# xujiabo/SCREAM

Hardware: AMD Instinct MI355X
Metric: registration pairs/sec (higher is better)
Workload: dtype f32; 1 GPU; BASELINE configs[1]: synthetic 3DMatch_test-like pairs, voxel 0.0625 m, ~5k points/cloud, batch-of-pairs=32 per GPU, A1-A10 per pair (forward 6+6 layers d_model 256, 1-NN thresh 0.1, Kabsch, RE/TE), random-init weights seed 0; lanes=1, steps_in_flight=2, parallelism=dp1 (pairs sharded, metric-row all-gather), rccl_ranks=1, gemm_backend=h2

## Files before the change

scream_amd/csrc/ring.h:

```cpp
#pragma once
#include "split.h"

namespace {

constexpr int T_PF = 3;

typedef const __attribute__((address_space(1))) void* gptr_t;
typedef __attribute__((address_space(3))) void* lptr_t;

constexpr int TT = 256;
constexpr int T_SLOTS = 3;
constexpr int T_MAX_GRID = SCREAM_MAX_GRID;

template <class SP> constexpr int stage_bytes() { return SP::NP * 16 * 1024; }
template <class SP> constexpr int wave_pieces() { return SP::NP * 4; }

template <int N>
__device__ __forceinline__ void ring_barrier() {
    __builtin_amdgcn_s_waitcnt(0x0070 | (N & 15) | ((N >> 4) << 14));
    __builtin_amdgcn_s_barrier();
}

__device__ __forceinline__ void lds_only_barrier() {
    __builtin_amdgcn_s_waitcnt(0xC07F);
    __builtin_amdgcn_s_barrier();
}

__host__ __device__ __forceinline__ int chunk_k(int s2, int half, int j) { return 8 * (2 * s2 + (j >> 2)) + 4 * half + (j & 3); }

__device__ __forceinline__ f32x4 ld4(const float* p) { return *reinterpret_cast<const f32x4*>(p); }

__device__ __forceinline__ void dma_1k(const char* src_lane, char* dst, int k) {
    switch (k) {
        case 0: __builtin_amdgcn_global_load_lds((gptr_t)src_lane, (lptr_t)dst, 16, 0, 0); break;
        case 1: __builtin_amdgcn_global_load_lds((gptr_t)src_lane, (lptr_t)dst, 16, 1024, 0); break;
        case 2: __builtin_amdgcn_global_load_lds((gptr_t)src_lane, (lptr_t)dst, 16, 2048, 0); break;
        default: __builtin_amdgcn_global_load_lds((gptr_t)src_lane, (lptr_t)dst, 16, 3072, 0); break;
    }
}

template <class V>
__device__ __forceinline__ V ld_frag(const char* p) {
    return *reinterpret_cast<const V*>(p);
}

template <class SP, int NV = 0>
__device__ __forceinline__ void mfma_group(f32x16& acc, const typename SP::vec (&w)[SP::NP], const typename SP::vec (&a)[SP::NP],
                                           bool zero = false) {
    f32x16 z;
#pragma unroll
    for (int e = 0; e < 16; ++e) z[e] = 0.f;
    SP::products(acc, w, a, zero ? z : acc);
    if (NV < 0) return;
    __builtin_amdgcn_sched_group_barrier(0x008, 1, 0);
    __builtin_amdgcn_sched_group_barrier(0x100, SP::NP, 0);
    if (NV == 0) {
        if (SP::NPROD > 1) __builtin_amdgcn_sched_group_barrier(0x008, SP::NPROD - 1, 0);
    } else {
#pragma unroll
        for (int i = 0; i < SP::NPROD - 1; ++i) {
            __builtin_amdgcn_sched_group_barrier(0x002, NV, 0);
            __builtin_amdgcn_sched_group_barrier(0x008, 1, 0);
        }
        __builtin_amdgcn_sched_group_barrier(0x002, NV, 0);
    }
    __builtin_amdgcn_sched_barrier(0);
}

template <int STEP, bool NT = false>
__device__ __forceinline__ void ld_asm4(f32x4 (&d)[4], const void* sbase, unsigned voff) {
    static_assert(STEP == 1024 || STEP == 32, "");
    if (STEP == 1024 && NT) {
        asm volatile("global_load_dwordx4 %0, %1, %2 nt" : "=v"(d[0]) : "v"(voff), "s"(sbase));
        asm volatile("global_load_dwordx4 %0, %1, %2 offset:1024 nt" : "=v"(d[1]) : "v"(voff), "s"(sbase));
        asm volatile("global_load_dwordx4 %0, %1, %2 offset:2048 nt" : "=v"(d[2]) : "v"(voff), "s"(sbase));
        asm volatile("global_load_dwordx4 %0, %1, %2 offset:3072 nt" : "=v"(d[3]) : "v"(voff), "s"(sbase));
    } else if (STEP == 1024) {
        asm volatile("global_load_dwordx4 %0, %1, %2" : "=v"(d[0]) : "v"(voff), "s"(sbase));
        asm volatile("global_load_dwordx4 %0, %1, %2 offset:1024" : "=v"(d[1]) : "v"(voff), "s"(sbase));
        asm volatile("global_load_dwordx4 %0, %1, %2 offset:2048" : "=v"(d[2]) : "v"(voff), "s"(sbase));
        asm volatile("global_load_dwordx4 %0, %1, %2 offset:3072" : "=v"(d[3]) : "v"(voff), "s"(sbase));
    } else {
        asm volatile("global_load_dwordx4 %0, %1, %2" : "=v"(d[0]) : "v"(voff), "s"(sbase));
        asm volatile("global_load_dwordx4 %0, %1, %2 offset:32" : "=v"(d[1]) : "v"(voff), "s"(sbase));
        asm volatile("global_load_dwordx4 %0, %1, %2 offset:64" : "=v"(d[2]) : "v"(voff), "s"(sbase));
        asm volatile("global_load_dwordx4 %0, %1, %2 offset:96" : "=v"(d[3]) : "v"(voff), "s"(sbase));
    }
}
__device__ __forceinline__ void ld_asm2k(f32x4& d0, f32x4& d1, const void* sbase, unsigned voff) {
    asm volatile("global_load_dwordx4 %0, %1, %2" : "=v"(d0) : "v"(voff), "s"(sbase));
    asm volatile("global_load_dwordx4 %0, %1, %2 offset:1024" : "=v"(d1) : "v"(voff), "s"(sbase));
}
__device__ __forceinline__ void pin(f32x4& v) { asm volatile("" : "+v"(v)); }

#define VM_WAIT(N) asm volatile("s_waitcnt vmcnt(" #N ")" ::: "memory")
template <int N>
__device__ __forceinline__ void vm_wait() {
    static_assert(N == 0 || N == 4 || N == 8 || N == 12, "");
    if (N == 0) VM_WAIT(0);
    else if (N == 4) VM_WAIT(4);
    else if (N == 8) VM_WAIT(8);
    else VM_WAIT(12);
}

}
```

scream_amd/csrc/split.h:

```cpp
#pragma once
#include "common.h"

namespace {

typedef __bf16 bf16x8 __attribute__((ext_vector_type(8)));
typedef _Float16 f16x8 __attribute__((ext_vector_type(8)));

struct SplitBf3 {
    static constexpr int NP = 3;
    static constexpr int NPROD = 6;
    static constexpr bool SCALED = false;
    typedef bf16x8 vec;
    static __device__ __forceinline__ void split1(float x, int i, vec (&p)[3]) {
        const __bf16 a = (__bf16)x;
        const float r1 = x - (float)a;
        const __bf16 b = (__bf16)r1;
        p[0][i] = a;
        p[1][i] = b;
        p[2][i] = (__bf16)(r1 - (float)b);
    }
    static __device__ __forceinline__ f32x16 mfma(vec a, vec b, f32x16 c) { return __builtin_amdgcn_mfma_f32_32x32x16_bf16(a, b, c, 0, 0, 0); }
    template <bool MIRROR = false>
    static __device__ __forceinline__ void products(f32x16& acc, const vec (&x)[3], const vec (&y)[3], const f32x16& c0) {
        if (MIRROR) {
            acc = mfma(x[2], y[0], c0);
            acc = mfma(x[1], y[1], acc);
            acc = mfma(x[0], y[2], acc);
            acc = mfma(x[1], y[0], acc);
            acc = mfma(x[0], y[1], acc);
        } else {
            acc = mfma(x[0], y[2], c0);
            acc = mfma(x[1], y[1], acc);
            acc = mfma(x[2], y[0], acc);
            acc = mfma(x[0], y[1], acc);
            acc = mfma(x[1], y[0], acc);
        }
        acc = mfma(x[0], y[0], acc);
    }
};

struct SplitH2 {
    static constexpr int NP = 2;
    static constexpr int NPROD = 3;
    static constexpr bool SCALED = true;
    typedef f16x8 vec;
    static __device__ __forceinline__ void split1(float x, int i, vec (&p)[2]) {
        const _Float16 a = (_Float16)x;
        p[0][i] = a;
        p[1][i] = (_Float16)(x - (float)a);
    }
    static __device__ __forceinline__ void split1s(float x, float s, int i, vec (&p)[2]) {
        const _Float16 a = (_Float16)__builtin_fmaf(x, s, 0.0f);
        p[0][i] = a;
        p[1][i] = (_Float16)__builtin_fmaf(x, s, -(float)a);
    }
    static __device__ __forceinline__ void split2s(float x0, float x1, float s, int i, vec (&p)[2]) {
        typedef unsigned u32x4 __attribute__((ext_vector_type(4)));
        unsigned hi, lo;
        asm("v_fma_mixlo_f16 %0, %1, %2, 0" : "=v"(hi) : "v"(x0), "v"(s));
        asm("v_fma_mixhi_f16 %0, %1, %2, 0" : "+v"(hi) : "v"(x1), "v"(s));
        asm("v_fma_mixlo_f16 %0, %1, %2, -%3 op_sel_hi:[0,0,1]" : "=v"(lo) : "v"(x0), "v"(s), "v"(hi));
        asm("v_fma_mixhi_f16 %0, %1, %2, -%3 op_sel:[0,0,1] op_sel_hi:[0,0,1]" : "+v"(lo) : "v"(x1), "v"(s), "v"(hi));
        u32x4 a = __builtin_bit_cast(u32x4, p[0]), b = __builtin_bit_cast(u32x4, p[1]);
        a[i >> 1] = hi;
        b[i >> 1] = lo;
        p[0] = __builtin_bit_cast(vec, a);
        p[1] = __builtin_bit_cast(vec, b);
    }
    static __device__ __forceinline__ void split1s_pair_here(float x, float y, float s, int i, vec (&p)[2], vec (&q)[2]) {
        typedef unsigned u32x4 __attribute__((ext_vector_type(4)));
        u32x4 pa = __builtin_bit_cast(u32x4, p[0]), pb = __builtin_bit_cast(u32x4, p[1]);
        u32x4 qa = __builtin_bit_cast(u32x4, q[0]), qb = __builtin_bit_cast(u32x4, q[1]);
        unsigned ph = pa[i >> 1], pl = pb[i >> 1], qh = qa[i >> 1], ql = qb[i >> 1];
        if ((i & 1) == 0) {
            asm volatile("v_fma_mixlo_f16 %0, %1, %2, 0" : "=v"(ph) : "v"(x), "s"(s));
            asm volatile("v_fma_mixlo_f16 %0, %1, %2, 0" : "=v"(qh) : "v"(y), "s"(s));
            asm volatile("v_fma_mixlo_f16 %0, %1, %2, -%3 op_sel_hi:[0,0,1]" : "=v"(pl) : "v"(x), "s"(s), "v"(ph));
            asm volatile("v_fma_mixlo_f16 %0, %1, %2, -%3 op_sel_hi:[0,0,1]" : "=v"(ql) : "v"(y), "s"(s), "v"(qh));
        } else {
            asm volatile("v_fma_mixhi_f16 %0, %1, %2, 0" : "+v"(ph) : "v"(x), "s"(s));
            asm volatile("v_fma_mixhi_f16 %0, %1, %2, 0" : "+v"(qh) : "v"(y), "s"(s));
            asm volatile("v_fma_mixhi_f16 %0, %1, %2, -%3 op_sel:[0,0,1] op_sel_hi:[0,0,1]" : "+v"(pl) : "v"(x), "s"(s), "v"(ph));
            asm volatile("v_fma_mixhi_f16 %0, %1, %2, -%3 op_sel:[0,0,1] op_sel_hi:[0,0,1]" : "+v"(ql) : "v"(y), "s"(s), "v"(qh));
        }
        pa[i >> 1] = ph;
        pb[i >> 1] = pl;
        qa[i >> 1] = qh;
        qb[i >> 1] = ql;
        p[0] = __builtin_bit_cast(vec, pa);
        p[1] = __builtin_bit_cast(vec, pb);
        q[0] = __builtin_bit_cast(vec, qa);
        q[1] = __builtin_bit_cast(vec, qb);
    }
    static __device__ __forceinline__ f32x16 mfma(vec a, vec b, f32x16 c) { return __builtin_amdgcn_mfma_f32_32x32x16_f16(a, b, c, 0, 0, 0); }
    template <bool MIRROR = false>
    static __device__ __forceinline__ void products(f32x16& acc, const vec (&x)[2], const vec (&y)[2], const f32x16& c0) {
        acc = mfma(x[0], y[1], c0);
        acc = mfma(x[1], y[0], acc);
        acc = mfma(x[0], y[0], acc);
    }
    static __device__ __forceinline__ f32x16 product(int i, const vec (&x)[2], const vec (&y)[2], const f32x16& c) {
        return i == 0 ? mfma(x[0], y[1], c) : i == 1 ? mfma(x[1], y[0], c) : mfma(x[0], y[0], c);
    }
};

struct SplitH1 {
    static constexpr int NP = 1;
    static constexpr int NPROD = 1;
    static constexpr bool SCALED = true;
    typedef f16x8 vec;
    static __device__ __forceinline__ void split1(float x, int i, vec (&p)[1]) { p[0][i] = (_Float16)x; }
    static __device__ __forceinline__ void split1s(float x, float s, int i, vec (&p)[1]) { p[0][i] = (_Float16)__builtin_fmaf(x, s, 0.0f); }
    static __device__ __forceinline__ void split2s(float x0, float x1, float s, int i, vec (&p)[1]) {
        split1s(x0, s, i, p);
        split1s(x1, s, i + 1, p);
    }
    static __device__ __forceinline__ f32x16 mfma(vec a, vec b, f32x16 c) { return __builtin_amdgcn_mfma_f32_32x32x16_f16(a, b, c, 0, 0, 0); }
    template <bool MIRROR = false>
    static __device__ __forceinline__ void products(f32x16& acc, const vec (&x)[1], const vec (&y)[1], const f32x16& c0) {
        acc = mfma(x[0], y[0], c0);
    }
    static __device__ __forceinline__ f32x16 product(int, const vec (&x)[1], const vec (&y)[1], const f32x16& c) { return mfma(x[0], y[0], c); }
};

template <class SP>
__device__ __forceinline__ void split8(const f32x4 lo, const f32x4 hi, typename SP::vec (&p)[SP::NP]) {
#pragma unroll
    for (int i = 0; i < 8; ++i) SP::split1(i < 4 ? lo[i] : hi[i - 4], i, p);
}

template <class SP>
__device__ __forceinline__ void split8s(const f32x4 lo, const f32x4 hi, float s, typename SP::vec (&p)[SP::NP]) {
    if constexpr (SP::SCALED) {
#pragma unroll
        for (int i = 0; i < 8; i += 2) SP::split2s(i < 4 ? lo[i] : hi[i - 4], i < 4 ? lo[i + 1] : hi[i - 3], s, i, p);
    } else {
        split8<SP>(lo, hi, p);
    }
}

static inline float exp2i(int e) {
    union { uint32_t u; float f; } v;
    v.u = (uint32_t)(e + 127) << 23;
    return v.f;
}

}
```

scream_amd/csrc/tail_split.hip:

```cpp
#include <type_traits>

#include "ring.h"

namespace {

constexpr int T_RIDE0 = 3;
constexpr int T_STASH = 3;
constexpr int T_DEFER_H2 = 2;

constexpr int TAIL_STAGES = 72;
constexpr int NEXT_Q_STAGES = 8;
constexpr int KV_PLANES_BYTES = 8 * 3 * 2 * 1024;
constexpr int KV_IMAGE_BYTES = KV_PLANES_BYTES + 8 * 32 * 4;

constexpr int KV_H2_HEAD_BYTES = 2 * 2 * 1024;
constexpr int KV_H2_SCALE_OFF = 8 * KV_H2_HEAD_BYTES;

struct HeadOps {
    f32x4 kv[6];
    f32x4 ks[4];
    f32x4 sc;
};

struct TailScales {
    float s_att;
    int e_q;
    int e_att;
    float c1;
    float eps1;
    float s_m1;
    float ch;
    float c2;
    float eps2;
    float s_y;
    float cq;
};

__device__ __forceinline__ constexpr int xadd_slot(int h, int g, int nd) {
    int n = 0;
    for (int c = 15 - nd; c >= 8; --c) {
        if ((c >> 1) == h - 1) continue;
        if (c == g) return n < 4 ? n : -1;
        ++n;
    }
    return -1;
}

template <class SP, bool NQ>
__global__ __launch_bounds__(TT, 1) void tail_kernel(const float* __restrict__ Q,
                                                     const char* __restrict__ kvimg,
                                                     const int32_t* __restrict__ tile_cloud, int kv_cloud_offset,
                                                     const int32_t* __restrict__ cloud_len,
                                                     const float* __restrict__ xres,
                                                     const char* __restrict__ Wimg,
                                                     const float* __restrict__ g1, const float* __restrict__ b1,
                                                     const float* __restrict__ g2, const float* __restrict__ b2,
                                                     float* __restrict__ y,
                                                     float* q_next,
                                                     int n_tiles, TailScales sc) {
    static_assert(!NQ || SP::SCALED, "the next-layer query projection is built for the fp16 splits");
    constexpr int N_STAGES = TAIL_STAGES + (NQ ? NEXT_Q_STAGES : 0);
    typedef typename SP::vec V;
    constexpr int NP = SP::NP;
    constexpr int STAGE = stage_bytes<SP>();
    constexpr int PIECES = wave_pieces<SP>();
    constexpr bool APPLY_H2 = SP::SCALED;
    constexpr int NV_MERGE = SP::NPROD >= 6 ? 6 : 8;
    constexpr int ND = SP::NPROD >= 6 ? 1 : T_DEFER_H2;
    constexpr int NG = 16 - ND;
    constexpr int NSTASH = NP == 2 ? T_STASH : 0;
    __shared__ __attribute__((aligned(16))) char smem[T_SLOTS * STAGE + 4096 + NSTASH * 16384];
    const int tid = threadIdx.x, lane = tid & 63;
    const int wave = __builtin_amdgcn_readfirstlane(tid >> 6);
    const int half = lane >> 5;
    float* lnp = reinterpret_cast<float*>(smem + T_SLOTS * STAGE);
    f32x4* stash = reinterpret_cast<f32x4*>(smem + T_SLOTS * STAGE + 4096 + wave * (NSTASH * 4096)) + lane;
    lnp[tid] = SP::SCALED ? g1[tid] * sc.s_m1 : g1[tid];
    lnp[256 + tid] = SP::SCALED ? b1[tid] * sc.s_m1 : b1[tid];
    lnp[512 + tid] = g2[tid];
    lnp[768 + tid] = b2[tid];
    const float eps1 = SP::SCALED ? sc.eps1 : 1e-5f, eps2 = SP::SCALED ? sc.eps2 : 1e-5f;
    const unsigned v_lane16 = lane * 16, v_half16 = half * 16;
    auto dma_piece = [&](unsigned q, int u) {
        const unsigned src = q % (unsigned)N_STAGES, slot = q % (unsigned)T_SLOTS;
        const char* sbase = Wimg + (size_t)src * STAGE + (wave * PIECES + (u & ~3)) * 1024;
        dma_1k(sbase + v_lane16, smem + slot * STAGE + (wave * PIECES + (u & ~3)) * 1024, u & 3);
    };
    unsigned q = 0;
#pragma unroll
    for (int u = 0; u < PIECES; ++u) dma_piece(0, u);
#pragma unroll
    for (int u = 0; u < PIECES; ++u) dma_piece(1, u);

    auto seg_base = [&](const float* base, int64_t grp, int seg) { return base + grp + seg * 1024; };
    auto req_q = [&](f32x4 (&qb)[4], int64_t grp, int h) {
        ld_asm4<1024, true>(qb, seg_base(Q, grp, h), v_lane16);
    };
    auto req_head = [&](HeadOps& o, const char* kvc, int h) {
        f32x4 (&kv4)[4] = reinterpret_cast<f32x4 (&)[4]>(o.kv[0]);
        if (APPLY_H2) {
            ld_asm4<1024>(kv4, kvc + h * KV_H2_HEAD_BYTES, v_lane16);
            asm volatile("global_load_dwordx4 %0, %1, %2" : "=v"(o.sc) : "v"(v_half16), "s"(kvc + KV_H2_SCALE_OFF + 32 * h));
        } else {
            const char* kp = kvc + h * (3 * 2 * 1024);
            ld_asm4<1024>(kv4, kp, v_lane16);
            ld_asm2k(o.kv[4], o.kv[5], kp + 4 * 1024, v_lane16);
        }
        ld_asm4<32>(o.ks, kvc + KV_PLANES_BYTES + 128 * h, v_half16);
    };
    auto req_x = [&](f32x4 (&xs)[4], int64_t grp, int blk, auto second) {
        ld_asm4<1024, decltype(second)::value>(xs, seg_base(xres, grp, blk), v_lane16);
    };
    auto pin_head = [&](HeadOps& o) {
#pragma unroll
        for (int a = 0; a < 4; ++a) pin(o.ks[a]);
#pragma unroll
        for (int f = 0; f < (APPLY_H2 ? 4 : 6); ++f) pin(o.kv[f]);
        if (APPLY_H2) pin(o.sc);
    };
    auto add_x4 = [&](f32x16& t, const f32x4 (&xs)[4], int a, float c) {
#pragma unroll
        for (int k = 0; k < 4; ++k) t[4 * a + k] = SP::SCALED ? __builtin_fmaf(xs[a][k], c, t[4 * a + k]) : t[4 * a + k] + xs[a][k];
    };
    auto pin_x = [&](f32x4 (&xs)[4]) {
#pragma unroll
        for (int a = 0; a < 4; ++a) pin(xs[a]);
    };
    auto add_x = [&](f32x16& t, const f32x4 (&xs)[4], float c) {
#pragma unroll
        for (int a = 0; a < 4; ++a) add_x4(t, xs, a, c);
    };

    HeadOps op;
    f32x4 qA[4], qB[4];
    f32x4 xs[4], xs2[4];
    V apA[2][NP], apB[2][NP];
    f32x16 aT;
    bf16x8 qp[2][3];
    f16x8 qph[2][2];
    float Zs = 0.f;
    int tq = 0;

    auto apply_qscale = [&](const f32x4 (&qb)[4]) {
        float m = 0.f;
#pragma unroll
        for (int a = 0; a < 4; ++a)
#pragma unroll
            for (int k = 0; k < 4; ++k) m = fmaxf(m, qb[a][k]);
        m = fmaxf(m, __shfl_xor(m, 32));
        const int hb = (int)(__float_as_uint(op.sc[0]) >> 23);
        tq = min(max(14 - ((int)(__float_as_uint(m) >> 23) - 127), sc.e_q), min(127, sc.e_att + hb - 1));
    };
    auto apply_qsplit = [&](f32x4 (&qb)[4], int s2) {
        const f32x4 lo = qb[2 * s2], hi = qb[2 * s2 + 1];
        if (APPLY_H2) split8s<SplitH2>(lo, hi, __uint_as_float((uint32_t)(tq + 127) << 23), qph[s2]);
        else split8<SplitBf3>(lo, hi, qp[s2]);
    };
    auto apply_mfma = [&](int s2) {
        if (APPLY_H2) {
            f16x8 w[2];
#pragma unroll
            for (int p = 0; p < 2; ++p) w[p] = __builtin_bit_cast(f16x8, op.kv[p * 2 + s2]);
            mfma_group<SplitH2, -1>(aT, w, qph[s2], s2 == 0);
        } else {
            bf16x8 w[3];
#pragma unroll
            for (int p = 0; p < 3; ++p) w[p] = __builtin_bit_cast(bf16x8, op.kv[p * 2 + s2]);
            mfma_group<SplitBf3, -1>(aT, w, qp[s2], s2 == 0);
        }
    };
    auto apply_z = [&](f32x4 (&qb)[4]) {
        float zp = 0.f;
#pragma unroll
        for (int a = 0; a < 4; ++a)
#pragma unroll
            for (int k = 0; k < 4; ++k) zp += qb[a][k] * op.ks[a][k];
        zp += __shfl_xor(zp, 32);
        Zs = 1.0f / (zp + 1e-6f);
        if (APPLY_H2) Zs *= __uint_as_float((uint32_t)(sc.e_att - tq + (int)(__float_as_uint(op.sc[0]) >> 23)) << 23);
        else if (SP::SCALED) Zs *= sc.s_att;
    };
    auto apply_split_pair = [&](int k, V (&ap)[2][NP], float S) {
        const int s2 = k >> 2, j = (2 * k) & 7;
#pragma unroll
        for (int e = 0; e < 2; ++e) SP::split1((aT[2 * k + e] * Zs) * S, j + e, ap[s2]);
    };
    auto apply_ride = [&](f32x4 (&qb)[4], int g, V (&ap)[2][NP], float S) {
        if (g == 0 && APPLY_H2) apply_qscale(qb);
        if (g == 0) apply_qsplit(qb, 0);
        if (g == 1) apply_qsplit(qb, 1);
        if (g == 1) apply_mfma(0);
        if (g == 2) apply_mfma(1);
        if (g == 3) apply_z(qb);
        if (g >= 4 && g < 12) apply_split_pair(g - 4, ap, S);
    };

    int tile = blockIdx.x;
    int64_t grp = ((int64_t)tile * 128 + wave * 32) * SCREAM_D_MODEL;
    const char* kvc = nullptr;
    float S = 1.f;
    if (tile < n_tiles) {
        const int cl = tile_cloud[tile] + kv_cloud_offset;
        kvc = kvimg + (size_t)cl * KV_IMAGE_BYTES;
        S = (float)cloud_len[cl];
    }
    if (tile < n_tiles) {
#pragma unroll
        for (int h = 0; h < 2; ++h) {
            req_q(qA, grp, h);
            req_head(op, kvc, h);
            VM_WAIT(0);
            pin_x(qA);
            pin_head(op);
#pragma unroll
            for (int g = 0; g < 12; ++g) apply_ride(qA, g, h == 0 ? apA : apB, S);
        }
    }

    while (tile < n_tiles) {
        V wfd[ND][NP];
        f32x16 acc[8];
        auto ring_groups = [&](auto flush, auto body) __attribute__((always_inline)) {
            const char* wb = smem + (q % T_SLOTS) * STAGE + lane * 16;
            V wf[T_PF][NP];
#pragma unroll
            for (int g0 = 0; g0 < T_PF - 1; ++g0)
#pragma unroll
                for (int p = 0; p < NP; ++p) wf[g0][p] = ld_frag<V>(wb + (p * 16 + g0) * 1024);
            flush();
#pragma unroll
            for (int g = 0; g < NG; ++g) {
                if (g + T_PF - 1 < 16) {
#pragma unroll
                    for (int p = 0; p < NP; ++p)
                        (g + T_PF - 1 >= NG ? wfd[g + T_PF - 1 - NG][p] : wf[(g + T_PF - 1) % T_PF][p]) = ld_frag<V>(wb + (p * 16 + g + T_PF - 1) * 1024);
                }
                body(g, wf[g % T_PF]);
            }
            ++q;
        };
        const int tile_next = tile + (int)gridDim.x;
        const bool has_next = tile_next < n_tiles;
        const int64_t grp_next = ((int64_t)(has_next ? tile_next : tile) * 128 + wave * 32) * SCREAM_D_MODEL;
        const char* kvc_next = kvc;
        float S_next = 1.f;
        if (has_next) {
            const int cl = tile_cloud[tile_next] + kv_cloud_offset;
            kvc_next = kvimg + (size_t)cl * KV_IMAGE_BYTES;
            S_next = (float)cloud_len[cl];
        }

        auto stage_merge = [&](auto hh, V (&ap)[2][NP], V (&ap_next)[2][NP], f32x4 (&q_cons)[4], f32x4 (&q_req)[4], auto flush) {
            constexpr int h = decltype(hh)::value;
            constexpr bool RIDE = h >= 1 && h <= 6;
            if (h == 0) { if (NQ) ring_barrier<0>(); else lds_only_barrier(); }
            else ring_barrier<PIECES>();
            __builtin_amdgcn_sched_barrier(0);
            f32x4 (&x_prev)[4] = (h & 1) ? xs : xs2;
            f32x4 (&x_req)[4] = (h & 1) ? xs2 : xs;
            if (h > 0) {
                pin_x(x_prev);
                if (h - 1 < NSTASH) {
#pragma unroll
                    for (int a = 0; a < 4; ++a) stash[((h - 1) * 4 + a) * 64] = x_prev[a];
                }
                if (RIDE) {
                    pin_head(op);
                    pin_x(q_cons);
                }
            }
            __builtin_amdgcn_sched_barrier(0);
            req_x(x_req, grp, h, std::false_type{});
            if (h + 2 < 8) req_q(q_req, grp, h + 2);
            if (h == 0) req_head(op, kvc, 2);
            __builtin_amdgcn_sched_barrier(0);
            ring_groups(flush, [&](int g, const V (&w)[NP]) __attribute__((always_inline)) {
                if (g == 4 && RIDE && h + 2 < 8) {
                    __builtin_amdgcn_sched_barrier(0);
                    req_head(op, kvc, h + 2);
                    __builtin_amdgcn_sched_barrier(0);
                }
                if (g >= 4 && g - 4 < PIECES) dma_piece(q + 2, g - 4);
                if (PIECES == 12 && g == 14) dma_piece(q + 2, 11);
                if (RIDE) apply_ride(q_cons, g, ap_next, S);
                if (h > 0) {
                    const int pc = xadd_slot(h, g, ND);
                    if (pc >= 0) add_x4(acc[h > 0 ? h - 1 : 0], x_prev, pc, sc.c1);
                }
                mfma_group<SP, (h > 0 ? NV_MERGE : 0)>(acc[g >> 1], w, ap[g & 1], h == 0 && (g & 1) == 0);
            });
        };
        constexpr std::integral_constant<bool, true> yes{};
        constexpr std::integral_constant<bool, false> no{};
#define HEAD(n) std::integral_constant<int, n>{}
        auto flush_none = [&]() {};
        auto flush_acc7 = [&](V (&b)[2][NP], bool first) {
#pragma unroll
            for (int i = 0; i < ND; ++i) mfma_group<SP, -1>(acc[7], wfd[i], b[(NG + i) & 1], first && ((NG + i) & 1) == 0);
        };
        auto flush_mergeA = [&]() { flush_acc7(apA, false); };
        auto flush_mergeB = [&]() { flush_acc7(apB, false); };
        auto flush_mergeA0 = [&]() { flush_acc7(apA, true); };
        stage_merge(HEAD(0), apA, apB, qB, qA, flush_none);
        stage_merge(HEAD(1), apB, apA, qA, qB, flush_mergeA0);
        stage_merge(HEAD(2), apA, apB, qB, qA, flush_mergeB);
        stage_merge(HEAD(3), apB, apA, qA, qB, flush_mergeA);
        stage_merge(HEAD(4), apA, apB, qB, qA, flush_mergeB);
        stage_merge(HEAD(5), apB, apA, qA, qB, flush_mergeA);
        stage_merge(HEAD(6), apA, apB, qB, qA, flush_mergeB);
        stage_merge(HEAD(7), apB, apA, qA, qB, flush_mergeA);
        flush_mergeB();
        vm_wait<PIECES>();
        pin_x(xs2);
        add_x(acc[7], xs2, sc.c1);

        V mp[16][NP];
        {
            float sum = 0.f;
#pragma unroll
            for (int b = 0; b < 8; ++b)
#pragma unroll
                for (int e = 0; e < 16; ++e) sum += acc[b][e];
            sum += __shfl_xor(sum, 32);
            const float mean = sum * (1.0f / 256.0f);
            float var = 0.f;
#pragma unroll
            for (int b = 0; b < 8; ++b)
#pragma unroll
                for (int e = 0; e < 16; ++e) {
                    acc[b][e] -= mean;
                    var += acc[b][e] * acc[b][e];
                }
            var += __shfl_xor(var, 32);
            const float rstd = 1.0f / sqrtf(var * (1.0f / 256.0f) + eps1);
            const float* gp = lnp + 4 * half;
            const float* bp = lnp + 256 + 4 * half;
#pragma unroll
            for (int b = 0; b < 8; ++b)
#pragma unroll
                for (int s2 = 0; s2 < 2; ++s2) {
                    f32x4 v[2];
#pragma unroll
                    for (int a2 = 0; a2 < 2; ++a2) {
                        const int a = 2 * s2 + a2;
                        const f32x4 g4 = ld4(gp + 32 * b + 8 * a), b4 = ld4(bp + 32 * b + 8 * a);
#pragma unroll
                        for (int k = 0; k < 4; ++k) v[a2][k] = acc[b][4 * a + k] * rstd * g4[k] + b4[k];
                    }
                    split8<SP>(v[0], v[1], mp[2 * b + s2]);
                }
        }

        f32x16 hT;
        V hpA[2][NP], hpB[2][NP];
        auto split_pair = [&](int k, V (&hout)[2][NP]) {
            const int s2 = k >> 2, j = (2 * k) & 7;
            float x0, x1;
            asm("v_max_f32 %0, 0, %1" : "=v"(x0) : "v"(hT[2 * k]));
            asm("v_max_f32 %0, 0, %1" : "=v"(x1) : "v"(hT[2 * k + 1]));
            if constexpr (SP::SCALED) {
                SP::split2s(x0, x1, sc.ch, j, hout[s2]);
            } else {
                SP::split1(x0, j, hout[s2]);
                SP::split1(x1, j + 1, hout[s2]);
            }
        };
        auto stage_up = [&](auto first, auto xload, auto flush) {
            constexpr int XLOAD = decltype(xload)::value;
            if (decltype(first)::value) ring_barrier<0>(); else ring_barrier<PIECES>();
            __builtin_amdgcn_sched_barrier(0);
            if (XLOAD >= 0 && XLOAD < NSTASH) {
#pragma unroll
                for (int a = 0; a < 4; ++a) xs[a] = stash[(XLOAD * 4 + a) * 64];
            } else if (XLOAD >= 0) req_x(xs, grp, XLOAD, std::true_type{});
            __builtin_amdgcn_sched_barrier(0);
            ring_groups(flush, [&](int g, const V (&w)[NP]) __attribute__((always_inline)) {
                if (g < PIECES) dma_piece(q + 2, g);
                mfma_group<SP>(hT, w, mp[g], g == 0);
            });
        };
        auto stage_down = [&](V (&hin)[2][NP], V (&hout)[2][NP], auto with_split, auto xadd, auto ride, auto flush) {
            constexpr int XADD = decltype(xadd)::value;
            constexpr int RIDE = decltype(ride)::value;
            ring_barrier<PIECES>();
            __builtin_amdgcn_sched_barrier(0);
            if (XADD == 0) {
                pin_x(xs);
#pragma unroll
                for (int a = 0; a < 4; ++a)
#pragma unroll
                    for (int k = 0; k < 4; ++k) acc[0][4 * a + k] = SP::SCALED ? xs[a][k] * sc.c2 : xs[a][k];
            } else if (XADD > 0) {
                pin_x(xs);
                add_x(acc[XADD > 0 ? XADD : 0], xs, sc.c2);
            }
            if (RIDE == 2) {
                pin_head(op);
                pin_x(qA);
            }
            __builtin_amdgcn_sched_barrier(0);
            if (RIDE == 1) {
                req_q(qA, grp_next, 0);
                req_head(op, kvc_next, 0);
            }
            __builtin_amdgcn_sched_barrier(0);
            ring_groups(flush, [&](int g, const V (&w)[NP]) __attribute__((always_inline)) {
                if (RIDE == 2 && g == 4) {
                    __builtin_amdgcn_sched_barrier(0);
                    req_q(qA, grp_next, 1);
                    req_head(op, kvc_next, 1);
                    __builtin_amdgcn_sched_barrier(0);
                }
                if (RIDE == 2) {
                    if (g >= 4 && g - 4 < PIECES) dma_piece(q + 2, g - 4);
                    if (PIECES == 12 && g == 14) dma_piece(q + 2, 11);
                } else {
                    if (g < PIECES) dma_piece(q + 2, g);
                }
                if (RIDE == 2) apply_ride(qA, g, apA, S_next);
                if (decltype(with_split)::value && (ND == 1 ? (g & 1) == 0 : (g >= T_RIDE0 && g < T_RIDE0 + 8))) split_pair(ND == 1 ? g >> 1 : g - T_RIDE0, hout);
                mfma_group<SP>(acc[g >> 1], w, hin[g & 1], XADD == 0 && g >= 2 && (g & 1) == 0);
            });
        };
        constexpr std::integral_constant<int, -1> none{};
        constexpr std::integral_constant<int, 0> ride0{};
        auto flush_up = [&]() {
#pragma unroll
            for (int i = 0; i < ND; ++i) mfma_group<SP, -1>(hT, wfd[i], mp[NG + i]);
        };
        auto flush_downA = [&]() { flush_acc7(hpA, false); };
        auto flush_downB = [&]() { flush_acc7(hpB, false); };
        auto flush_downA0 = [&]() { flush_acc7(hpA, true); };
        stage_up(yes, none, flush_none);
        flush_up();
#pragma unroll
        for (int k = 0; k < 8; ++k) split_pair(k, hpA);
#define PAIR(c, fl, flA)                                                                    \
        stage_up(no, HEAD((c) - 1), fl);                                        \
        stage_down(hpA, hpB, yes, HEAD((c) - 1), ride0, flush_up);  \
        stage_up(no, HEAD(c), flA);                                         \
        stage_down(hpB, hpA, yes, HEAD(c), ride0, flush_up);
        PAIR(1, flush_none, flush_downA0) PAIR(3, flush_downB, flush_downA) PAIR(5, flush_downB, flush_downA) PAIR(7, flush_downB, flush_downA)
#undef PAIR
        for (int c = 9; c < 31; c += 2) {
            stage_up(no, none, flush_downB);
            stage_down(hpA, hpB, yes, none, ride0, flush_up);
            stage_up(no, none, flush_downA);
            stage_down(hpB, hpA, yes, none, ride0, flush_up);
        }
        stage_up(no, none, flush_downB);
        stage_down(hpA, hpB, yes, none, HEAD(1), flush_up);
        stage_down(hpB, hpA, no, none, HEAD(2), flush_downA);
        flush_downB();
#undef HEAD
        VM_WAIT(0);
        if (has_next) {
            pin_head(op);
            pin_x(qA);
#pragma unroll
            for (int g = 0; g < 12; ++g) apply_ride(qA, g, apB, S_next);
        }

        V yp[NQ ? 16 : 1][NP];
        {
            float sum = 0.f;
#pragma unroll
            for (int b = 0; b < 8; ++b)
#pragma unroll
                for (int e = 0; e < 16; ++e) sum += acc[b][e];
            sum += __shfl_xor(sum, 32);
            const float mean = sum * (1.0f / 256.0f);
            float var = 0.f;
#pragma unroll
            for (int b = 0; b < 8; ++b)
#pragma unroll
                for (int e = 0; e < 16; ++e) {
                    acc[b][e] -= mean;
                    var += acc[b][e] * acc[b][e];
                }
            var += __shfl_xor(var, 32);
            const float rstd = 1.0f / sqrtf(var * (1.0f / 256.0f) + eps2);
            const float* gp = lnp + 512 + 4 * half;
            const float* bp = lnp + 768 + 4 * half;
            float* yg = y + grp + lane * 4;
#pragma unroll
            for (int b = 0; b < 8; ++b)
#pragma unroll
                for (int s2 = 0; s2 < 2; ++s2) {
                    f32x4 o2[2];
#pragma unroll
                    for (int a2 = 0; a2 < 2; ++a2) {
                        const int a = 2 * s2 + a2;
                        const f32x4 g4 = ld4(gp + 32 * b + 8 * a), b4 = ld4(bp + 32 * b + 8 * a);
                        f32x4 o;
#pragma unroll
                        for (int k = 0; k < 4; ++k) o[k] = acc[b][4 * a + k] * rstd * g4[k] + b4[k];
                        __builtin_nontemporal_store(o, reinterpret_cast<f32x4*>(yg + (b * 4 + a) * 256));
                        o2[a2] = o;
                    }
                    if (NQ) split8<SP>(o2[0] * sc.s_y, o2[1] * sc.s_y, yp[NQ ? 2 * b + s2 : 0]);
                }
        }
        if constexpr (NQ) {
            f32x16 hq[2];
            f32x4 oq[4];
            float* qg = q_next + grp + lane * 4;
            auto elu_pair = [&](int k, const f32x16& h) {
#pragma unroll
                for (int e = 0; e < 2; ++e) {
                    const int i = 2 * k + e;
                    const float x = h[i] * sc.cq;
                    oq[i >> 2][i & 3] = elu1(x);
                }
            };
            auto store_chunk = [&](int j) {
#pragma unroll
                for (int a = 0; a < 4; ++a) __builtin_nontemporal_store(oq[a], reinterpret_cast<f32x4*>(qg + (j * 4 + a) * 256));
            };
            constexpr int PP = (PIECES + NG - 9) / (NG - 8);
            auto stage_q = [&](auto jj) {
                constexpr int j = decltype(jj)::value;
                if (j == 0) lds_only_barrier(); else ring_barrier<PIECES>();
                __builtin_amdgcn_sched_barrier(0);
                auto flush_q = [&]() {
                    if (j > 0) {
#pragma unroll
                        for (int i = 0; i < ND; ++i) mfma_group<SP, -1>(hq[(j + 1) & 1], wfd[i], yp[NG + i]);
                    }
                };
                ring_groups(flush_q, [&](int g, const V (&w)[NP]) __attribute__((always_inline)) {
                    if (j > 0 && g < 8) elu_pair(g, hq[(j + 1) & 1]);
                    if (g == 8) {
                        __builtin_amdgcn_sched_barrier(0);
                        if (j > 0) store_chunk(j - 1);
                        __builtin_amdgcn_sched_barrier(0);
                    }
                    if (g >= 8) {
#pragma unroll
                        for (int u = (g - 8) * PP; u < (g - 7) * PP; ++u)
                            if (u < PIECES) dma_piece(q + 2, u);
                    }
                    mfma_group<SP, 8>(hq[j & 1], w, yp[g], g == 0);
                });
            };
            stage_q(std::integral_constant<int, 0>{});
            stage_q(std::integral_constant<int, 1>{});
            stage_q(std::integral_constant<int, 2>{});
            stage_q(std::integral_constant<int, 3>{});
            stage_q(std::integral_constant<int, 4>{});
            stage_q(std::integral_constant<int, 5>{});
            stage_q(std::integral_constant<int, 6>{});
            stage_q(std::integral_constant<int, 7>{});
#pragma unroll
            for (int i = 0; i < ND; ++i) mfma_group<SP, -1>(hq[1], wfd[i], yp[NG + i]);
#pragma unroll
            for (int k = 0; k < 8; ++k) elu_pair(k, hq[1]);
            store_chunk(7);
        }
        tile = tile_next;
        grp = ((int64_t)tile_next * 128 + wave * 32) * SCREAM_D_MODEL;
        kvc = kvc_next;
        S = S_next;
    }
    VM_WAIT(0);
}

__global__ __launch_bounds__(256) void act_layout_kernel(const float* __restrict__ src, float* __restrict__ dst, int to_frag) {
    __shared__ float tile[32][260];
    const int t = threadIdx.x;
    const float* s = src + (int64_t)blockIdx.x * 8192;
    float* d = dst + (int64_t)blockIdx.x * 8192;
#pragma unroll
    for (int i = 0; i < 8; ++i) {
        const int e = t + 256 * i;
        const f32x4 v = *reinterpret_cast<const f32x4*>(s + e * 4);
        int row, col;
        if (to_frag) {
            row = e >> 6, col = (e & 63) * 4;
        } else {
            const int ln = e & 63, a = (e >> 6) & 3, blk = e >> 8;
            row = ln & 31, col = 32 * blk + 8 * a + 4 * (ln >> 5);
        }
        *reinterpret_cast<f32x4*>(&tile[row][col]) = v;
    }
    __syncthreads();
#pragma unroll
    for (int i = 0; i < 8; ++i) {
        const int e = t + 256 * i;
        int row, col;
        if (to_frag) {
            const int ln = e & 63, a = (e >> 6) & 3, blk = e >> 8;
            row = ln & 31, col = 32 * blk + 8 * a + 4 * (ln >> 5);
        } else {
            row = e >> 6, col = (e & 63) * 4;
        }
        *reinterpret_cast<f32x4*>(d + e * 4) = *reinterpret_cast<const f32x4*>(&tile[row][col]);
    }
}

template <class SP>
__global__ void pack_tail_kernel(const float* __restrict__ Wm, const float* __restrict__ W1, const float* __restrict__ W2,
                                 const float* __restrict__ Wq_next, float s_wm, float s_w1, float s_w2, float s_wq,
                                 typename SP::vec* __restrict__ out) {
    const int t = blockIdx.x * blockDim.x + threadIdx.x;
    if (t >= (TAIL_STAGES + (Wq_next ? NEXT_Q_STAGES : 0)) * 16 * 64) return;
    const int lane = t & 63, frag = (t >> 6) & 15, stage = t >> 10;
    const int m = lane & 31, half = lane >> 5;
    float v[8];
    float s;
    if (stage < 8) {
        s = s_wm;
#pragma unroll
        for (int j = 0; j < 8; ++j) v[j] = Wm[(int64_t)(32 * (frag >> 1) + m) * 256 + 32 * stage + chunk_k(frag & 1, half, j)];
    } else if (stage >= TAIL_STAGES) {
        s = s_wq;
#pragma unroll
        for (int j = 0; j < 8; ++j) v[j] = Wq_next[(int64_t)(32 * (stage - TAIL_STAGES) + m) * 256 + 32 * (frag >> 1) + chunk_k(frag & 1, half, j)];
    } else {
        const int st = stage - 8;
        const bool up = st == 0 || (st < 63 && (st & 1));
        const int c = st == 0 ? 0 : st == 63 ? 31 : up ? (st + 1) / 2 : st / 2 - 1;
        s = up ? s_w1 : s_w2;
        if (up) {
#pragma unroll
            for (int j = 0; j < 8; ++j) v[j] = W1[(int64_t)(32 * c + m) * 256 + 32 * (frag >> 1) + chunk_k(frag & 1, half, j)];
        } else {
#pragma unroll
            for (int j = 0; j < 8; ++j) v[j] = W2[(int64_t)(32 * (frag >> 1) + m) * 1024 + 32 * c + chunk_k(frag & 1, half, j)];
        }
    }
    typename SP::vec p[SP::NP];
#pragma unroll
    for (int j = 0; j < 8; ++j) SP::split1(SP::SCALED ? v[j] * s : v[j], j, p);
#pragma unroll
    for (int pl = 0; pl < SP::NP; ++pl) out[(((int64_t)stage * SP::NP + pl) * 16 + frag) * 64 + lane] = p[pl];
}

constexpr int KVF_THREADS = 320;

template <bool H2>
__global__ __launch_bounds__(KVF_THREADS) void kv_finalize_image_kernel(const float* __restrict__ partial,
                                                                      const int32_t* __restrict__ cloud_row0,
                                                                      const int32_t* __restrict__ cloud_len, int64_t row_base,
                                                                      int cloud_begin, char* __restrict__ kvimg,
                                                                      int64_t partial_layer_stride, int64_t image_layer_stride) {
    constexpr int KV_ELEMS = (SCREAM_HEAD_DIM + 1) * SCREAM_HEAD_DIM;
    static_assert(KV_ELEMS % 4 == 0 && KV_ELEMS / 4 <= KVF_THREADS, "");
    __shared__ float wmax[KVF_THREADS / 64];
    const int i4 = threadIdx.x;
    const bool active = i4 < KV_ELEMS / 4;
    const int kvi = blockIdx.x / SCREAM_NHEAD, h = blockIdx.x % SCREAM_NHEAD;
    const int cloud = cloud_begin + kvi;
    partial += (int64_t)blockIdx.y * partial_layer_stride;
    kvimg += (int64_t)blockIdx.y * image_layer_stride;
    const int t0 = (int)((cloud_row0[cloud] - row_base) / SCREAM_ROW_TILE);
    const int nt = (cloud_len[cloud] + SCREAM_ROW_TILE - 1) / SCREAM_ROW_TILE;
    const float* p = partial + ((int64_t)t0 * SCREAM_NHEAD + h) * KV_ELEMS + 4 * (active ? i4 : 0);
    char* img = kvimg + (size_t)cloud * KV_IMAGE_BYTES;
    const float S = (float)cloud_len[cloud];
    f32x4 s8[16];
#pragma unroll
    for (int u = 0; u < 16; ++u) s8[u] = f32x4{0.f, 0.f, 0.f, 0.f};
    if (active) {
        for (int c = 0; c < nt; c += 16) {
#pragma unroll
            for (int u = 0; u < 16; ++u)
                if (c + u < nt) s8[u] += *reinterpret_cast<const f32x4*>(p + (int64_t)(c + u) * SCREAM_NHEAD * KV_ELEMS);
        }
    }
#pragma unroll
    for (int u = 0; u < 8; ++u) s8[u] += s8[u + 8];
    const f32x4 s4 = ((s8[0] + s8[1]) + (s8[2] + s8[3])) + ((s8[4] + s8[5]) + (s8[6] + s8[7]));
    const bool is_kv = 4 * i4 < 32 * 32;
    f32x4 x4;
#pragma unroll
    for (int e = 0; e < 4; ++e) x4[e] = s4[e] / S;
    float scale = 1.f;
    if (H2) {
        float m = (active && is_kv) ? fmaxf(fmaxf(fabsf(x4[0]), fabsf(x4[1])), fmaxf(fabsf(x4[2]), fabsf(x4[3]))) : 0.f;
#pragma unroll
        for (int o = 32; o >= 1; o >>= 1) m = fmaxf(m, __shfl_xor(m, o));
        if ((threadIdx.x & 63) == 0) wmax[threadIdx.x >> 6] = m;
        __syncthreads();
        m = wmax[0];
#pragma unroll
        for (int w = 1; w < KVF_THREADS / 64; ++w) m = fmaxf(m, wmax[w]);
        const uint32_t mb = __float_as_uint(m);
        int eh = 15 - ((int)(mb >> 23) - 127) - ((mb & 0x7fffffu) ? 1 : 0);
        if (!(m >= 1.17549435e-38f) || eh > 40) eh = 40;
        if (eh < -30) eh = -30;
        scale = __uint_as_float((uint32_t)(eh + 127) << 23);
        if (threadIdx.x < 8) reinterpret_cast<float*>(img + KV_H2_SCALE_OFF)[h * 8 + threadIdx.x] = __uint_as_float((uint32_t)(127 - eh) << 23);
    }
    if (!active) return;
#pragma unroll
    for (int e = 0; e < 4; ++e) {
        const int i = 4 * i4 + e;
        if (is_kv) {
            const int d = i >> 5, v = i & 31;
            const float x = x4[e];
            const int s2 = d >> 4, hf = (d >> 2) & 1, j = 4 * ((d >> 3) & 1) + (d & 3);
            if (H2) {
                const _Float16 a = (_Float16)(x * scale);
                const _Float16 b = (_Float16)__builtin_fmaf(x, scale, -(float)a);
                _Float16* base = reinterpret_cast<_Float16*>(img) + ((size_t)(h * 2) * 2 + s2) * 512 + (v + 32 * hf) * 8 + j;
                base[0] = a;
                base[2 * 512] = b;
            } else {
                const __bf16 a = (__bf16)x;
                const float r1 = x - (float)a;
                const __bf16 b = (__bf16)r1;
                const __bf16 cc = (__bf16)(r1 - (float)b);
                __bf16* base = reinterpret_cast<__bf16*>(img) + ((size_t)(h * 3) * 2 + s2) * 512 + (v + 32 * hf) * 8 + j;
                base[0] = a;
                base[2 * 512] = b;
                base[4 * 512] = cc;
            }
        } else {
            reinterpret_cast<float*>(img + KV_PLANES_BYTES)[h * 32 + (i - 32 * 32)] = s4[e];
        }
    }
}

bool split_ok(int32_t split) { return split == SCREAM_SPLIT_BF3 || split == SCREAM_SPLIT_H2 || split == SCREAM_SPLIT_H1; }

bool tail_scales(const scream_tail_exps_t* ex, TailScales* sc) {
    if (!ex) return false;
    const int es[6] = {ex->e_att, ex->e_wm, ex->e_m1, ex->e_w1, ex->e_h, ex->e_w2};
    for (int e : es)
        if (e < -40 || e > 40) return false;
    const int e1 = ex->e_wm + ex->e_att, e2 = ex->e_w2 + ex->e_h, eh = ex->e_h - ex->e_w1 - ex->e_m1;
    if (e1 < -44 || e1 > 44 || e2 < -44 || e2 > 44 || eh < -100 || eh > 100) return false;
    if (ex->e_q < -40 || ex->e_q > 40) return false;
    sc->s_att = exp2i(ex->e_att);
    sc->e_q = ex->e_q;
    sc->e_att = ex->e_att;
    sc->c1 = exp2i(e1);
    sc->eps1 = 1e-5f * exp2i(2 * e1);
    sc->s_m1 = exp2i(ex->e_m1);
    sc->ch = exp2i(eh);
    sc->c2 = exp2i(e2);
    sc->eps2 = 1e-5f * exp2i(2 * e2);
    if (ex->e_y < -40 || ex->e_y > 40 || ex->e_wq < -40 || ex->e_wq > 40) return false;
    sc->s_y = exp2i(ex->e_y);
    sc->cq = exp2i(-ex->e_y - ex->e_wq);
    return true;
}

}

extern "C" int64_t scream_tail_image_bytes(int32_t split, int32_t with_next_q) {
    if (!split_ok(split) || (with_next_q && split == SCREAM_SPLIT_BF3)) return SCREAM_EINVAL;
    return (int64_t)(TAIL_STAGES + (with_next_q ? NEXT_Q_STAGES : 0)) * split * 16 * 1024;
}
extern "C" int64_t scream_kv_image_bytes(void) { return KV_IMAGE_BYTES; }

extern "C" int scream_pack_tail(const float* Wm, const float* W1, const float* W2, const float* Wq_next, int32_t split,
                                const scream_tail_exps_t* exps, void* image, void* stream) {
    SCREAM_REQUIRE(Wm && W1 && W2 && image && split_ok(split), SCREAM_EINVAL);
    SCREAM_REQUIRE(!Wq_next || split != SCREAM_SPLIT_BF3, SCREAM_EUNSUPPORTED);
    SCREAM_REQUIRE((reinterpret_cast<uintptr_t>(image) & 15) == 0, SCREAM_EINVAL);
    const dim3 grid((TAIL_STAGES + (Wq_next ? NEXT_Q_STAGES : 0)) * 16 * 64 / 256), block(256);
    if (split != SCREAM_SPLIT_BF3) {
        TailScales sc;
        SCREAM_REQUIRE(tail_scales(exps, &sc), SCREAM_EINVAL);
        if (split == SCREAM_SPLIT_H2)
            pack_tail_kernel<SplitH2><<<grid, block, 0, as_stream(stream)>>>(Wm, W1, W2, Wq_next, exp2i(exps->e_wm), exp2i(exps->e_w1),
                                                                             exp2i(exps->e_w2), exp2i(exps->e_wq), reinterpret_cast<f16x8*>(image));
        else
            pack_tail_kernel<SplitH1><<<grid, block, 0, as_stream(stream)>>>(Wm, W1, W2, Wq_next, exp2i(exps->e_wm), exp2i(exps->e_w1),
                                                                             exp2i(exps->e_w2), exp2i(exps->e_wq), reinterpret_cast<f16x8*>(image));
    } else {
        pack_tail_kernel<SplitBf3><<<grid, block, 0, as_stream(stream)>>>(Wm, W1, W2, nullptr, 1.f, 1.f, 1.f, 1.f, reinterpret_cast<bf16x8*>(image));
    }
    SCREAM_LAUNCH_CHECK();
    return 0;
}

extern "C" int scream_kv_finalize_image(const float* kv_partial, const int32_t* cloud_row0, const int32_t* cloud_len,
                                        int64_t row_base, int32_t cloud_begin, int32_t n_kv, void* kv_image, int32_t n_layers,
                                        int64_t partial_layer_stride, int64_t image_layer_stride, int32_t split, void* stream) {
    SCREAM_REQUIRE(kv_partial && cloud_row0 && cloud_len && kv_image && split_ok(split), SCREAM_EINVAL);
    SCREAM_REQUIRE(n_kv >= 0 && cloud_begin >= 0 && row_base >= 0 && n_layers >= 1 && n_layers <= 65535, SCREAM_EINVAL);
    SCREAM_REQUIRE(n_layers == 1 || (partial_layer_stride > 0 && image_layer_stride > 0 && image_layer_stride % 16 == 0), SCREAM_EINVAL);
    SCREAM_REQUIRE(((reinterpret_cast<uintptr_t>(kv_image) | reinterpret_cast<uintptr_t>(kv_partial)) & 15) == 0 && partial_layer_stride % 4 == 0,
                   SCREAM_EINVAL);
    if (n_kv == 0) return 0;
    const dim3 grid(n_kv * SCREAM_NHEAD, n_layers), block(KVF_THREADS);
    if (split != SCREAM_SPLIT_BF3)
        kv_finalize_image_kernel<true><<<grid, block, 0, as_stream(stream)>>>(kv_partial, cloud_row0, cloud_len, row_base, cloud_begin,
                                                                              reinterpret_cast<char*>(kv_image), partial_layer_stride, image_layer_stride);
    else
        kv_finalize_image_kernel<false><<<grid, block, 0, as_stream(stream)>>>(kv_partial, cloud_row0, cloud_len, row_base, cloud_begin,
                                                                               reinterpret_cast<char*>(kv_image), partial_layer_stride, image_layer_stride);
    SCREAM_LAUNCH_CHECK();
    return 0;
}

namespace {
template <class SP, bool NQ>
void launch_tail(unsigned grid, hipStream_t st, const float* Q, const void* kv_image, const int32_t* tile_cloud, int32_t kv_cloud_offset,
                 const int32_t* cloud_len, const float* x, const void* tail_image, const float* g1, const float* b1, const float* g2,
                 const float* b2, float* y, float* q_next, int tiles, const TailScales& sc) {
    tail_kernel<SP, NQ><<<dim3(grid), dim3(TT), 0, st>>>(Q, reinterpret_cast<const char*>(kv_image), tile_cloud, kv_cloud_offset, cloud_len, x,
                                                     reinterpret_cast<const char*>(tail_image), g1, b1, g2, b2, y, q_next, tiles, sc);
}
}

extern "C" int scream_layer_tail_f32(const float* Q, const void* kv_image, const int32_t* tile_cloud,
                                     int32_t kv_cloud_offset, const int32_t* cloud_len, const float* x,
                                     const void* tail_image, const float* g1, const float* b1, const float* g2,
                                     const float* b2, float* y, float* q_next, int64_t M, int32_t split,
                                     const scream_tail_exps_t* exps, void* stream) {
    SCREAM_REQUIRE(Q && kv_image && tile_cloud && cloud_len && x && tail_image && g1 && b1 && g2 && b2 && y && split_ok(split), SCREAM_EINVAL);
    SCREAM_REQUIRE(M >= 0 && M % SCREAM_ROW_TILE == 0, SCREAM_EUNSUPPORTED);
    SCREAM_REQUIRE(((reinterpret_cast<uintptr_t>(Q) | reinterpret_cast<uintptr_t>(kv_image) | reinterpret_cast<uintptr_t>(x) |
                     reinterpret_cast<uintptr_t>(tail_image) | reinterpret_cast<uintptr_t>(g1) | reinterpret_cast<uintptr_t>(b1) |
                     reinterpret_cast<uintptr_t>(g2) | reinterpret_cast<uintptr_t>(b2) | reinterpret_cast<uintptr_t>(y) |
                     reinterpret_cast<uintptr_t>(q_next)) & 15) == 0, SCREAM_EINVAL);
    SCREAM_REQUIRE(x != y, SCREAM_EINVAL);
    SCREAM_REQUIRE(!q_next || (split != SCREAM_SPLIT_BF3 && q_next != x && q_next != y), SCREAM_EINVAL);
    TailScales sc{1.f, 0, 0, 1.f, 1e-5f, 1.f, 1.f, 1.f, 1e-5f, 1.f, 1.f};
    if (split != SCREAM_SPLIT_BF3) SCREAM_REQUIRE(tail_scales(exps, &sc), SCREAM_EINVAL);
    const int64_t tiles = M / SCREAM_ROW_TILE;
    if (tiles == 0) return 0;
    SCREAM_REQUIRE(tiles < (1ll << 31), SCREAM_EUNSUPPORTED);
    const unsigned grid = tiles < T_MAX_GRID ? (unsigned)tiles : (unsigned)T_MAX_GRID;
    hipStream_t st = as_stream(stream);
#define TAIL_ARGS grid, st, Q, kv_image, tile_cloud, kv_cloud_offset, cloud_len, x, tail_image, g1, b1, g2, b2, y, q_next, (int)tiles, sc
    if (split == SCREAM_SPLIT_H2) {
        if (q_next) launch_tail<SplitH2, true>(TAIL_ARGS);
        else launch_tail<SplitH2, false>(TAIL_ARGS);
    } else if (split == SCREAM_SPLIT_H1) {
        if (q_next) launch_tail<SplitH1, true>(TAIL_ARGS);
        else launch_tail<SplitH1, false>(TAIL_ARGS);
    } else {
        launch_tail<SplitBf3, false>(TAIL_ARGS);
    }
#undef TAIL_ARGS
    SCREAM_LAUNCH_CHECK();
    return 0;
}

extern "C" int scream_act_layout(const float* src, float* dst, int64_t M, int32_t to_fragment, void* stream) {
    SCREAM_REQUIRE(src && dst && src != dst, SCREAM_EINVAL);
    SCREAM_REQUIRE(M >= 0 && M % 32 == 0 && M / 32 < (1ll << 31), SCREAM_EUNSUPPORTED);
    SCREAM_REQUIRE(((reinterpret_cast<uintptr_t>(src) | reinterpret_cast<uintptr_t>(dst)) & 15) == 0, SCREAM_EINVAL);
    if (M == 0) return 0;
    act_layout_kernel<<<dim3((unsigned)(M / 32)), dim3(256), 0, as_stream(stream)>>>(src, dst, to_fragment ? 1 : 0);
    SCREAM_LAUNCH_CHECK();
    return 0;
}
```

Before: 1895 pairs/s.

## Interleave H2 split, x-add and fragment loads between individual MFMAs

For the SplitH2 backend, the down stage now issues each MFMA product separately, fenced by scheduling barriers. It slots the next fragment LDS loads, DMA issue, the residual x-add into the accumulators and a staged f16 hi/lo split of the activations between those MFMAs. The deferred flush products in flush_up get the same per-product placement. The goal is to hide VALU and LDS latency under the matrix pipe instead of running them as separate bursts. In exchange the compiler loses scheduling freedom, register pressure rises, and the hand ordering may stall if the dependencies are placed too tightly.

```diff
diff --git a/scream_amd/csrc/ring.h b/scream_amd/csrc/ring.h
--- a/scream_amd/csrc/ring.h
+++ b/scream_amd/csrc/ring.h
@@ -67,6 +67,18 @@
     __builtin_amdgcn_sched_barrier(0);
 }
 
+template <class SP, class Mfma, class Behind>
+__device__ __forceinline__ void mfma_group_placed(Mfma&& mfma, Behind&& behind) {
+#pragma unroll
+    for (int m = 0; m < SP::NPROD; ++m) {
+        __builtin_amdgcn_sched_barrier(0);
+        mfma(m);
+        __builtin_amdgcn_sched_barrier(0);
+        behind(m);
+    }
+    __builtin_amdgcn_sched_barrier(0);
+}
+
 template <int STEP, bool NT = false>
 __device__ __forceinline__ void ld_asm4(f32x4 (&d)[4], const void* sbase, unsigned voff) {
     static_assert(STEP == 1024 || STEP == 32, "");
diff --git a/scream_amd/csrc/split.h b/scream_amd/csrc/split.h
--- a/scream_amd/csrc/split.h
+++ b/scream_amd/csrc/split.h
@@ -37,6 +37,10 @@
         }
         acc = mfma(x[0], y[0], acc);
     }
+    static __device__ __forceinline__ f32x16 product(int i, const vec (&x)[3], const vec (&y)[3], const f32x16& c) {
+        return i == 0 ? mfma(x[0], y[2], c) : i == 1 ? mfma(x[1], y[1], c) : i == 2 ? mfma(x[2], y[0], c)
+             : i == 3 ? mfma(x[0], y[1], c) : i == 4 ? mfma(x[1], y[0], c) : mfma(x[0], y[0], c);
+    }
 };
 
 struct SplitH2 {
@@ -66,6 +70,22 @@
         b[i >> 1] = lo;
         p[0] = __builtin_bit_cast(vec, a);
         p[1] = __builtin_bit_cast(vec, b);
+    }
+    static __device__ __forceinline__ void split2s_step(int step, float x0, float x1, float s, unsigned& hi, unsigned& lo, int i, vec (&p)[2]) {
+        typedef unsigned u32x4 __attribute__((ext_vector_type(4)));
+        if (step == 0) {
+            asm volatile("v_fma_mixlo_f16 %0, %1, %2, 0" : "=v"(hi) : "v"(x0), "v"(s));
+        } else if (step == 1) {
+            asm volatile("v_fma_mixlo_f16 %0, %1, %2, -%3 op_sel_hi:[0,0,1]" : "=v"(lo) : "v"(x0), "v"(s), "v"(hi));
+            asm volatile("v_fma_mixhi_f16 %0, %1, %2, 0" : "+v"(hi) : "v"(x1), "v"(s));
+        } else {
+            asm volatile("v_fma_mixhi_f16 %0, %1, %2, -%3 op_sel:[0,0,1] op_sel_hi:[0,0,1]" : "+v"(lo) : "v"(x1), "v"(s), "v"(hi));
+            u32x4 a = __builtin_bit_cast(u32x4, p[0]), b = __builtin_bit_cast(u32x4, p[1]);
+            a[i >> 1] = hi;
+            b[i >> 1] = lo;
+            p[0] = __builtin_bit_cast(vec, a);
+            p[1] = __builtin_bit_cast(vec, b);
+        }
     }
     static __device__ __forceinline__ void split1s_pair_here(float x, float y, float s, int i, vec (&p)[2], vec (&q)[2]) {
         typedef unsigned u32x4 __attribute__((ext_vector_type(4)));
diff --git a/scream_amd/csrc/tail_split.hip b/scream_amd/csrc/tail_split.hip
--- a/scream_amd/csrc/tail_split.hip
+++ b/scream_amd/csrc/tail_split.hip
@@ -68,6 +68,7 @@
     constexpr int NV_MERGE = SP::NPROD >= 6 ? 6 : 8;
     constexpr int ND = SP::NPROD >= 6 ? 1 : T_DEFER_H2;
     constexpr int NG = 16 - ND;
+    constexpr bool PLACED = std::is_same<SP, SplitH2>::value;
     constexpr int NSTASH = NP == 2 ? T_STASH : 0;
     __shared__ __attribute__((aligned(16))) char smem[T_SLOTS * STAGE + 4096 + NSTASH * 16384];
     const int tid = threadIdx.x, lane = tid & 63;
@@ -239,6 +240,28 @@
             }
             ++q;
         };
+        auto ring_groups_placed = [&](auto flush, auto fride, auto mfma, auto ride) __attribute__((always_inline)) {
+            const char* wb = smem + (q % T_SLOTS) * STAGE + lane * 16;
+            V wf[T_PF][NP];
+#pragma unroll
+            for (int g0 = 0; g0 < T_PF - 1; ++g0)
+#pragma unroll
+                for (int p = 0; p < NP; ++p) wf[g0][p] = ld_frag<V>(wb + (p * 16 + g0) * 1024);
+            flush(fride);
+#pragma unroll
+            for (int g = 0; g < NG; ++g) {
+                mfma_group_placed<SP>([&](int m) __attribute__((always_inline)) { mfma(g, m, wf[g % T_PF]); },
+                                      [&](int m) __attribute__((always_inline)) {
+                    if (m == 0 && g + T_PF - 1 < 16) {
+#pragma unroll
+                        for (int p = 0; p < NP; ++p)
+                            (g + T_PF - 1 >= NG ? wfd[g + T_PF - 1 - NG][p] : wf[(g + T_PF - 1) % T_PF][p]) = ld_frag<V>(wb + (p * 16 + g + T_PF - 1) * 1024);
+                    }
+                    ride(g, m);
+                });
+            }
+            ++q;
+        };
         const int tile_next = tile + (int)gridDim.x;
         const bool has_next = tile_next < n_tiles;
         const int64_t grp_next = ((int64_t)(has_next ? tile_next : tile) * 128 + wave * 32) * SCREAM_D_MODEL;
@@ -365,6 +388,21 @@
                 SP::split1(x1, j + 1, hout[s2]);
             }
         };
+        float sp_x0 = 0.f, sp_x1 = 0.f;
+        unsigned sp_hi = 0, sp_lo = 0;
+        auto split_pair_step = [&](int k, int m, V (&hout)[2][NP]) __attribute__((always_inline)) {
+            if constexpr (std::is_same<SP, SplitH2>::value) {
+                if (m == 1) {
+                    if (k < 8) asm volatile("v_max_f32 %0, 0, %1" : "=v"(sp_x0) : "v"(hT[2 * k]));
+                    if (k >= 1) SP::split2s_step(2, sp_x0, sp_x1, sc.ch, sp_hi, sp_lo, (2 * (k - 1)) & 7, hout[(k - 1) >> 2]);
+                    if (k < 8) {
+                        asm volatile("v_max_f32 %0, 0, %1" : "=v"(sp_x1) : "v"(hT[2 * k + 1]));
+                        SP::split2s_step(0, sp_x0, sp_x1, sc.ch, sp_hi, sp_lo, (2 * k) & 7, hout[k >> 2]);
+                    }
+                }
+                if (m == 2 && k < 8) SP::split2s_step(1, sp_x0, sp_x1, sc.ch, sp_hi, sp_lo, (2 * k) & 7, hout[k >> 2]);
+            }
+        };
         auto stage_up = [&](auto first, auto xload, auto flush) {
             constexpr int XLOAD = decltype(xload)::value;
             if (decltype(first)::value) ring_barrier<0>(); else ring_barrier<PIECES>();
@@ -384,15 +422,18 @@
             constexpr int RIDE = decltype(ride)::value;
             ring_barrier<PIECES>();
             __builtin_amdgcn_sched_barrier(0);
+            constexpr bool PLACED_HERE = PLACED && RIDE != 2;
             if (XADD == 0) {
                 pin_x(xs);
-#pragma unroll
-                for (int a = 0; a < 4; ++a)
-#pragma unroll
-                    for (int k = 0; k < 4; ++k) acc[0][4 * a + k] = SP::SCALED ? xs[a][k] * sc.c2 : xs[a][k];
+                if (!PLACED_HERE) {
+#pragma unroll
+                    for (int a = 0; a < 4; ++a)
+#pragma unroll
+                        for (int k = 0; k < 4; ++k) acc[0][4 * a + k] = SP::SCALED ? xs[a][k] * sc.c2 : xs[a][k];
+                }
             } else if (XADD > 0) {
                 pin_x(xs);
-                add_x(acc[XADD > 0 ? XADD : 0], xs, sc.c2);
+                if (!PLACED_HERE) add_x(acc[XADD > 0 ? XADD : 0], xs, sc.c2);
             }
             if (RIDE == 2) {
                 pin_head(op);
@@ -404,6 +445,34 @@
                 req_head(op, kvc_next, 0);
             }
             __builtin_amdgcn_sched_barrier(0);
+            if constexpr (PLACED_HERE) {
+                auto xadd_elems = [&](int e0, int e1) __attribute__((always_inline)) {
+                    f32x16& t = acc[XADD > 0 ? XADD : 0];
+#pragma unroll
+                    for (int e = e0; e < e1; ++e) {
+                        float r = XADD == 0 ? xs[e >> 2][e & 3] * sc.c2 : __builtin_fmaf(xs[e >> 2][e & 3], sc.c2, t[e]);
+                        asm volatile("" : "+a"(r));
+                        t[e] = r;
+                    }
+                };
+                constexpr int NF = ND * SP::NPROD;
+                auto xadd_flush = [&](int i) __attribute__((always_inline)) {
+                    if (XADD == 0) xadd_elems((i * 16 + NF - 1) / NF, ((i + 1) * 16 + NF - 1) / NF);
+                    else if (XADD > 0) xadd_elems(2 * i, 2 * i + 2);
+                };
+                f32x16 z;
+#pragma unroll
+                for (int e = 0; e < 16; ++e) z[e] = 0.f;
+                ring_groups_placed(flush, xadd_flush,
+                    [&](int g, int m, const V (&w)[NP]) __attribute__((always_inline)) {
+                        acc[g >> 1] = SP::product(m, w, hin[g & 1], XADD == 0 && g >= 2 && (g & 1) == 0 && m == 0 ? z : acc[g >> 1]);
+                    },
+                    [&](int g, int m) __attribute__((always_inline)) {
+                        if (XADD > 0 && g < 2 && m == 1) xadd_elems(2 * (NF + g), 2 * (NF + g) + 2);
+                        if (decltype(with_split)::value && g >= T_RIDE0 && g <= T_RIDE0 + 8) split_pair_step(g - T_RIDE0, m, hout);
+                        if (m == 0 && g < PIECES) dma_piece(q + 2, g);
+                    });
+            } else
             ring_groups(flush, [&](int g, const V (&w)[NP]) __attribute__((always_inline)) {
                 if (RIDE == 2 && g == 4) {
                     __builtin_amdgcn_sched_barrier(0);
@@ -424,9 +493,16 @@
         };
         constexpr std::integral_constant<int, -1> none{};
         constexpr std::integral_constant<int, 0> ride0{};
-        auto flush_up = [&]() {
-#pragma unroll
-            for (int i = 0; i < ND; ++i) mfma_group<SP, -1>(hT, wfd[i], mp[NG + i]);
+        auto flush_up = [&](auto... fr) __attribute__((always_inline)) {
+#pragma unroll
+            for (int i = 0; i < ND; ++i) {
+                if constexpr (sizeof...(fr) == 0) {
+                    mfma_group<SP, -1>(hT, wfd[i], mp[NG + i]);
+                } else {
+                    mfma_group_placed<SP>([&](int m) __attribute__((always_inline)) { hT = SP::product(m, wfd[i], mp[NG + i], hT); },
+                                          [&](int m) __attribute__((always_inline)) { (fr(i * SP::NPROD + m), ...); });
+                }
+            }
         };
         auto flush_downA = [&]() { flush_acc7(hpA, false); };
         auto flush_downB = [&]() { flush_acc7(hpB, false); };
```

Result: no change. 1905 pairs/s (median of 6 runs) (+0.6%).
